# INK-USC/RE-Net

Hardware: AMD Instinct MI355X
Metric: RGCN+GRU encoder triples/s at bs=1024 n_hidden=200 (full training step, both directions) (higher is better)
Workload: dtype f32; 1 GPU; ICEWS18-shaped synthetic stream (seed 999), n_hidden=200, seq_len=10, batch=1024 per GPU, dropout=0.50, fwd+bwd both directions + clip + Adam; parallelism=dp1, global_batch=1024, nodes=99312, edges=288792

## Files before the change

### include/renet_hip.h

```cpp
#ifndef RENET_HIP_H
#define RENET_HIP_H

#include <stddef.h>
#include <stdint.h>

#ifdef __cplusplus
extern "C" {
#endif

#define RENET_OK 0
#define RENET_ERR_BADARG (-1)
#define RENET_ERR_UNSUPPORTED (-2)
#define RENET_ERR_WORKSPACE (-3)

#define RENET_ABI_VERSION 1
int renet_version(void);

int renet_gather_rows(const float* table, const int32_t* idx, int n, int D, float* out, void* stream);
int renet_segment_add(const float* src, const int32_t* order, const int32_t* seg_ptr,
                      const int32_t* seg_target, int U, int D, float* dst, void* stream);
int renet_segment_add2(const float* src0, const float* src1, const int32_t* order, const int32_t* seg_ptr,
                       const int32_t* seg_target, int U, int D, float* dst0, float* dst1, void* stream);

int renet_rgcn_gather(const float* x, int D, const int32_t* row_ptr, const int32_t* col,
// ... 114 lines not shown
                           const int32_t* subj_row, const int32_t* row_ent, const int32_t* row_rel,
                           const int32_t* glob_row, int S, int D, float drop_p, uint64_t seed_x,
                           uint64_t seed_xr, float* X, float* Xr, void* stream);
int renet_bound_parts(size_t total4);
int renet_seq_assemble_fwd_bounds(const float* h2, const float* ent, const float* rel, const float* glob,
                                  const int32_t* subj_row, const int32_t* row_ent, const int32_t* row_rel,
                                  const int32_t* glob_row, int S, int D, float drop_p, uint64_t seed_x,
                                  uint64_t seed_xr, float* X, float* Xr, float* partX, float* partXr, void* stream);
int renet_seq_assemble_bwd(const float* dX, const float* dXr, const int32_t* step_off, int L, int S,
                           int B, int D, float drop_p, uint64_t seed_x, uint64_t seed_xr, float* dRows,
                           float* dEntSeq, float* dRelSeq, void* stream);

size_t renet_gru_workspace(int B, int H);
int renet_gru_fwd(const float* Gi, const int32_t* step_off, int L, int H, const float* Whh,
                  const float* bhh, float* h_last, int out_rows, float* saved, float* workspace,
                  size_t workspace_bytes, void* stream);
int renet_gru_bwd(const float* dh_last, const int32_t* step_off, int L, int H, const float* Whh,
                  const float* saved, float* dGi, float* dGh, float* workspace,
                  size_t workspace_bytes, void* stream);
int renet_gru_fwd_multi(int n, const float* const* Gi, const int32_t* step_off, int L, int H,
                        const float* const* Whh, const float* const* bhh, float* const* h_last, int out_rows,
                        float* const* saved, float* workspace, size_t workspace_bytes, void* stream);
int renet_gru_bwd_multi(int n, const float* const* dh_last, const int32_t* step_off, int L, int H,
                        const float* const* Whh, const float* const* saved, float* const* dGi,
                        float* const* dGh, float* workspace, size_t workspace_bytes, void* stream);
int renet_gru_fwd_layouts(int n, const float* const* Gi, const int32_t* const* step_off, const int* L, int H,
                          const float* const* Whh, const float* const* bhh, float* const* h_last,
                          const int* out_rows, float* const* saved, float* workspace, size_t workspace_bytes,
                          void* stream);
int renet_gru_bwd_layouts(int n, const float* const* dh_last, const int32_t* const* step_off, const int* L, int H,
                          const float* const* Whh, const float* const* saved, float* const* dGi,
                          float* const* dGh, float* workspace, size_t workspace_bytes, void* stream);
int renet_gru_bound_parts(int max_rows);
int renet_gru_bwd_layouts_bounds(int n, const float* const* dh_last, const int32_t* const* step_off, const int* L, int H,
                                 const float* const* Whh, const float* const* saved, float* const* dGi,
                                 float* const* dGh, float* const* bounds, float* workspace, size_t workspace_bytes,
                                 void* stream);
int renet_gru_fwd_layouts_f32(int n, const float* const* Gi, const int32_t* const* step_off, const int* L, int H,
                              const float* const* Whh, const float* const* bhh, float* const* h_last,
                              const int* out_rows, float* const* saved, float* workspace, size_t workspace_bytes,
                              void* stream);
int renet_gru_bwd_layouts_f32(int n, const float* const* dh_last, const int32_t* const* step_off, const int* L, int H,
                              const float* const* Whh, const float* const* saved, float* const* dGi,
                              float* const* dGh, float* workspace, size_t workspace_bytes, void* stream);
int renet_gru_fwd_layouts_bf16(int n, const float* const* Gi, const int32_t* const* step_off, const int* L, int H,
                               const float* const* Whh, const float* const* bhh, float* const* h_last,
                               const int* out_rows, float* const* saved, float* workspace, size_t workspace_bytes,
                               void* stream);
int renet_gru_bwd_layouts_bf16(int n, const float* const* dh_last, const int32_t* const* step_off, const int* L, int H,
                               const float* const* Whh, const float* const* saved, float* const* dGi,
                               float* const* dGh, float* workspace, size_t workspace_bytes, void* stream);

int renet_concat3_fwd(const float* a, const int32_t* ia, const float* hmid, const float* c,
                      const int32_t* ic, int B, int D, float drop_p, uint64_t seed, float* feat,
                      void* stream);
int renet_concat3_fwd_bounds(const float* a, const int32_t* ia, const float* hmid, const float* c,
                             const int32_t* ic, int B, int D, float drop_p, uint64_t seed, float* feat,
                             float* bound_part, void* stream);
int renet_concat3_bwd(const float* dfeat, int B, int D, int parts, float drop_p, uint64_t seed,
                      float* da_rows, float* dhmid, float* dc_rows, void* stream);
int renet_dropout(const float* x, size_t n, float drop_p, uint64_t seed, float* y, void* stream);
int renet_softmax_ce(const float* logits, const int32_t* target, int B, int C, int ld,
                     float grad_scale, float* row_loss, float* dlogits, void* stream);

int renet_segment_pool_fwd(const float* h, const int32_t* seg_ptr, int G, int D, int is_max,
                           float* out, int32_t* argmax, void* stream);
int renet_segment_pool_bwd(const float* dout, const int32_t* seg_ptr, const int32_t* argmax, int G,
                           int D, int is_max, int N, float* dh, void* stream);

size_t renet_adam_workspace(size_t n);
int renet_adam_step(float* p, float* g, float* m, float* v, size_t n, float lr, float beta1, float beta2,
                    float eps, float weight_decay, float max_norm, int step, int zero_grad, float* workspace,
                    size_t workspace_bytes, float* grad_norm_out, void* stream);
int renet_adam_step_scaled(float* p, float* g, float* m, float* v, size_t n, float lr, float beta1, float beta2,
                           float eps, float weight_decay, float max_norm, float grad_scale, int step,
                           int zero_grad, float* workspace, size_t workspace_bytes, float* grad_norm_out,
                           void* stream);

int renet_sumsq_partials(const float* g, size_t n, float* partial, int n_slots, void* stream);
int renet_adam_step_presummed(float* p, float* g, float* m, float* v, size_t n, float lr, float beta1, float beta2,
                              float eps, float weight_decay, float max_norm, float grad_scale, int step, int zero_grad,
                              const float* partial, int n_partial, float* grad_norm_out, void* stream);

int renet_joint_softmax(float* logits, int ld, int n, int R, int N, const float* logits_r, int ld_r,
                        const float* prob_e, void* stream);
size_t renet_topk_workspace(int n);
int renet_topk_positive(const float* x, size_t ldx, int n, int M, int k, float* out_val, int64_t* out_idx,
                        void* workspace, size_t workspace_bytes, void* stream);

int renet_rank_rows(const float* scores, int ld, int n, int C, const int32_t* label, const int32_t* filt_ptr,
                    const int32_t* filt_col, int filtered, int32_t* greater, int32_t* equal, float* row_loss,
                    void* stream);

typedef struct {
    const int32_t *q_s, *q_r, *q_o;
    const int32_t* h_first[2];
    const int32_t* h_count[2];
    const int32_t* snap_t[2];
    const int32_t* snap_ptr[2];
    const int32_t* nbr_o[2];
    const int32_t* times;
    const int32_t* trip_ptr;
    const int32_t *trip_s, *trip_r, *trip_o;
    const int32_t* glob_times;
    int T, n_glob, n_facts, num_ent, num_rels;
} RenetStoreDev;

typedef struct {
    int32_t *node_ent, *node_slot, *row_ptr, *col, *etype;
    float* norm;
    int32_t *heavy_rows, *e_src, *e_dst, *chunk_ptr, *chunk_type, *type_chunk_ptr;
    int32_t *e_src2, *e_dst2, *chunk_ptr2, *chunk_type2, *type_chunk_ptr2;
    int32_t *it_src, *it_type, *grp_ptr;
    int32_t *subj_row, *row_seq, *row_ent, *row_rel, *glob_row;
    int32_t *s_sorted, *r_sorted, *rel_label, *ent_label, *perm, *step_off;
    int32_t* plan_order[4];
    int32_t* plan_seg[4];
    int32_t* plan_target[4];
    int32_t* counts;
    int cap_nodes, cap_edges;
    int32_t* seg_ptr;
} RenetBatchOut;

enum {
    RENET_BB_NNZ = 0, RENET_BB_S, RENET_BB_L, RENET_BB_TB, RENET_BB_FACTS, RENET_BB_N, RENET_BB_NA, RENET_BB_E2,
    RENET_BB_E, RENET_BB_NHEAVY, RENET_BB_NHEAVY_OUT, RENET_BB_NCHUNKS, RENET_BB_NCHUNKS2, RENET_BB_NITEMS,
    RENET_BB_NGROUPS, RENET_BB_NGROUPS_OUT, RENET_BB_NSEG0, RENET_BB_NSEG1, RENET_BB_NSEG2, RENET_BB_NSEG3,
    RENET_BB_ERR, RENET_BB_EOUT,
    RENET_BB_STEP_OFF = 24,
    RENET_BB_NCOUNTS = 64
};
enum { RENET_BB_ERR_TIME = 1, RENET_BB_ERR_GLOB = 2, RENET_BB_ERR_NODES = 4, RENET_BB_ERR_EDGES = 8 };

size_t renet_build_batch_workspace(const RenetStoreDev* store, int B, int cap_nodes, int cap_edges);
int renet_build_batch_both(const RenetStoreDev* store, const int32_t* idx_dev, int B, int seq_len, int heavy_thresh,
                           int group_budget, int chunk, const RenetBatchOut* out, void* workspace,
                           size_t workspace_bytes, void* stream);

typedef struct {
    const int32_t* node_ptr;
    const int32_t* node_ent_all;
    const int32_t* trip_ptr;
    const int32_t *trip_ls, *trip_r, *trip_lo;
    int T, n_nodes, n_facts, num_ent, num_rels;
} RenetFullStoreDev;

size_t renet_build_full_graphs_workspace(const RenetFullStoreDev* store, int G, int cap_nodes, int cap_edges);
int renet_build_full_graphs(const RenetFullStoreDev* store, const int32_t* tidx_dev, int G, int heavy_thresh,
                            int group_items, int chunk, RenetBatchOut* out, void* workspace, size_t workspace_bytes,
                            void* stream);

typedef struct { const int32_t *order, *seg_ptr, *target; int num_segments; } RenetSegPlan;
typedef struct {
    int D, num_ent, T, C2;
    float drop_p;
    const float *ent, *rel;
    const float *w1, *loop1, *w2, *loop2;
    const float *wih, *whh, *bih, *bhh;
    const float *wih_r, *whh_r, *bih_r, *bhh_r;
    const float *lin_w, *lin_b;
    const float *linr_w, *linr_b;
    float *g_ent, *g_rel, *g_w1, *g_loop1, *g_w2, *g_loop2, *g_wih, *g_whh, *g_bih, *g_bhh, *g_wih_r, *g_whh_r, *g_bih_r,
          *g_bhh_r, *g_lin_w, *g_lin_b, *g_linr_w, *g_linr_b;
    const float* glob;
    const void* lin_w_planes;
    size_t lin_w_plane;
// ... 64 lines not shown
```

### re-net_amd/csrc/optim.hip

```cpp
#include "common.h"

namespace {

constexpr int kBlocks = 2048;

__global__ __launch_bounds__(256) void sumsq_partial_kernel(const float4* __restrict__ g, size_t n4,
                                                            const float* __restrict__ g_tail, int tail,
                                                            float* __restrict__ partial) {
    __shared__ float red[4];
    float s = 0.f;
    for (size_t i = (size_t)blockIdx.x * 256 + threadIdx.x; i < n4; i += (size_t)gridDim.x * 256) {
        const float4 v = g[i];
        s += (v.x * v.x + v.y * v.y) + (v.z * v.z + v.w * v.w);
    }
    if (blockIdx.x == 0 && (int)threadIdx.x < tail) s += g_tail[threadIdx.x] * g_tail[threadIdx.x];
#pragma unroll
    for (int o = 32; o > 0; o >>= 1) s += __shfl_xor(s, o);
    if ((threadIdx.x & 63) == 0) red[threadIdx.x >> 6] = s;
    __syncthreads();
    if (threadIdx.x == 0) partial[blockIdx.x] = (red[0] + red[1]) + (red[2] + red[3]);
}

struct AdamCfg {
    float lr, beta1, beta2, eps, wd, max_norm, bc1, bc2_sqrt;
    float grad_scale;
    int zero_grad;
};

__device__ __forceinline__ float adam_one(float& p, float g, float& m, float& v, const AdamCfg& c, float coef) {
    g = g * coef + c.wd * p;
    m = c.beta1 * m + (1.f - c.beta1) * g;
    v = c.beta2 * v + (1.f - c.beta2) * g * g;
    const float denom = sqrtf(v) / c.bc2_sqrt + c.eps;
    p -= (c.lr / c.bc1) * (m / denom);
    return 0.f;
}

__global__ __launch_bounds__(256) void adam_kernel(float* __restrict__ p, float* __restrict__ g,
                                                   float* __restrict__ m, float* __restrict__ v, size_t n,
                                                   const float* __restrict__ partial, int n_partial, AdamCfg c,
                                                   float* __restrict__ norm_out) {
    __shared__ float red[4];
    __shared__ float s_coef;
    float s = 0.f;
    for (int i = threadIdx.x; i < n_partial; i += 256) s += partial[i];
#pragma unroll
    for (int o = 32; o > 0; o >>= 1) s += __shfl_xor(s, o);
    if ((threadIdx.x & 63) == 0) red[threadIdx.x >> 6] = s;
    __syncthreads();
    if (threadIdx.x == 0) {
        const float norm = c.grad_scale * sqrtf((red[0] + red[1]) + (red[2] + red[3]));
        float coef = 1.f;
        if (c.max_norm > 0.f) coef = fminf(c.max_norm / (norm + 1e-6f), 1.f);
        s_coef = coef * c.grad_scale;
        if (blockIdx.x == 0 && norm_out) *norm_out = norm;
    }
    __syncthreads();
    const float coef = s_coef;
    const size_t n4 = n / 4;
    float4* p4 = reinterpret_cast<float4*>(p);
    float4* g4 = reinterpret_cast<float4*>(g);
    float4* m4 = reinterpret_cast<float4*>(m);
    float4* v4 = reinterpret_cast<float4*>(v);
    for (size_t i = (size_t)blockIdx.x * 256 + threadIdx.x; i < n4; i += (size_t)gridDim.x * 256) {
        float4 pp = p4[i], gg = g4[i], mm = m4[i], vv = v4[i];
        adam_one(pp.x, gg.x, mm.x, vv.x, c, coef);
        adam_one(pp.y, gg.y, mm.y, vv.y, c, coef);
        adam_one(pp.z, gg.z, mm.z, vv.z, c, coef);
        adam_one(pp.w, gg.w, mm.w, vv.w, c, coef);
        p4[i] = pp; m4[i] = mm; v4[i] = vv;
        if (c.zero_grad) g4[i] = make_float4(0.f, 0.f, 0.f, 0.f);
    }
    if (blockIdx.x == 0 && threadIdx.x < (n & 3)) {
        const size_t i = n4 * 4 + threadIdx.x;
        float pp = p[i], mm = m[i], vv = v[i];
        adam_one(pp, g[i], mm, vv, c, coef);
        p[i] = pp; m[i] = mm; v[i] = vv;
        if (c.zero_grad) g[i] = 0.f;
    }
}

}

extern "C" {

size_t renet_adam_workspace(size_t n) {
    (void)n;
    return kBlocks * sizeof(float);
}

int renet_adam_step(float* p, float* g, float* m, float* v, size_t n, float lr, float beta1, float beta2,
                    float eps, float weight_decay, float max_norm, int step, int zero_grad, float* workspace,
                    size_t workspace_bytes, float* grad_norm_out, void* stream) {
    return renet_adam_step_scaled(p, g, m, v, n, lr, beta1, beta2, eps, weight_decay, max_norm, 1.f, step, zero_grad,
                                  workspace, workspace_bytes, grad_norm_out, stream);
}

int renet_sumsq_partials(const float* g, size_t n, float* partial, int n_slots, void* stream) {
    if (!g || !partial || n_slots < 1 || n_slots > kBlocks) return RENET_ERR_BADARG;
    if (reinterpret_cast<uintptr_t>(g) & 15) return RENET_ERR_BADARG;
    const size_t n4 = n / 4;
    RENET_LAUNCH(sumsq_partial_kernel, dim3(n_slots), dim3(256), 0, (hipStream_t)stream, (const float4*)g, n4, g + n4 * 4,
                       (int)(n & 3), partial);
    RENET_LAUNCH_CHECK();
    return RENET_OK;
}

static int adam_launch(float* p, float* g, float* m, float* v, size_t n, float lr, float beta1, float beta2, float eps,
                       float weight_decay, float max_norm, float grad_scale, int step, int zero_grad, const float* partial,
                       int n_partial, float* grad_norm_out, hipStream_t st) {
    const size_t n4 = n / 4;
    const int blocks = (int)max((size_t)1, min((size_t)kBlocks, (n4 + 255) / 256));
    AdamCfg c;
    c.lr = lr; c.beta1 = beta1; c.beta2 = beta2; c.eps = eps; c.wd = weight_decay; c.max_norm = max_norm;
    c.bc1 = 1.f - powf(beta1, (float)step);
    c.bc2_sqrt = sqrtf(1.f - powf(beta2, (float)step));
    c.zero_grad = zero_grad;
    c.grad_scale = grad_scale;
    RENET_LAUNCH(adam_kernel, dim3(blocks), dim3(256), 0, st, p, g, m, v, n, partial, n_partial, c, grad_norm_out);
    RENET_LAUNCH_CHECK();
    return RENET_OK;
}

int renet_adam_step_presummed(float* p, float* g, float* m, float* v, size_t n, float lr, float beta1, float beta2,
                              float eps, float weight_decay, float max_norm, float grad_scale, int step, int zero_grad,
                              const float* partial, int n_partial, float* grad_norm_out, void* stream) {
    if (step < 1 || lr < 0.f || beta1 < 0.f || beta1 >= 1.f || beta2 < 0.f || beta2 >= 1.f) return RENET_ERR_BADARG;
    if (n == 0) return RENET_OK;
    if (!partial || n_partial < 1 || n_partial > kBlocks) return RENET_ERR_BADARG;
    if ((reinterpret_cast<uintptr_t>(p) | reinterpret_cast<uintptr_t>(g) | reinterpret_cast<uintptr_t>(m) |
         reinterpret_cast<uintptr_t>(v)) & 15) return RENET_ERR_BADARG;
    return adam_launch(p, g, m, v, n, lr, beta1, beta2, eps, weight_decay, max_norm, grad_scale, step, zero_grad, partial,
                       n_partial, grad_norm_out, (hipStream_t)stream);
}

int renet_adam_step_scaled(float* p, float* g, float* m, float* v, size_t n, float lr, float beta1, float beta2,
                           float eps, float weight_decay, float max_norm, float grad_scale, int step, int zero_grad,
                           float* workspace, size_t workspace_bytes, float* grad_norm_out, void* stream) {
    if (step < 1 || lr < 0.f || beta1 < 0.f || beta1 >= 1.f || beta2 < 0.f || beta2 >= 1.f) return RENET_ERR_BADARG;
    if (n == 0) return RENET_OK;
    if (workspace_bytes < renet_adam_workspace(n)) return RENET_ERR_WORKSPACE;
    if ((reinterpret_cast<uintptr_t>(p) | reinterpret_cast<uintptr_t>(g) | reinterpret_cast<uintptr_t>(m) |
         reinterpret_cast<uintptr_t>(v)) & 15) return RENET_ERR_BADARG;
    hipStream_t st = (hipStream_t)stream;
    const size_t n4 = n / 4;
    const int blocks = (int)max((size_t)1, min((size_t)kBlocks, (n4 + 255) / 256));
    RENET_LAUNCH(sumsq_partial_kernel, dim3(blocks), dim3(256), 0, st, (const float4*)g, n4, g + n4 * 4,
                       (int)(n & 3), workspace);
    RENET_LAUNCH_CHECK();
    return adam_launch(p, g, m, v, n, lr, beta1, beta2, eps, weight_decay, max_norm, grad_scale, step, zero_grad, workspace,
                       blocks, grad_norm_out, st);
}


}
```

### re-net_amd/parallel.py

```python
import os

import torch
import torch.distributed as dist


def flat_layout(params):
    offs, off = [], 0
    for p in params:
        offs.append(off)
        off += (p.numel() + 3) & ~3
    return offs, off


def ordered_params(module, first=()):
    ps = [p for p in module.parameters() if p.requires_grad]
    own = {id(p) for p in ps}
    front, seen = [], set()
    for p in first:
        if id(p) in own and id(p) not in seen:
            front.append(p)
            seen.add(id(p))
    return front + [p for p in ps if id(p) not in seen]


# ... 211 lines not shown
        self.partials_ready = self._done_regions == set(r for r in self.regions() if r[1]) and \
            (self.sumsq_fn is not None or self.stream is None)
        if self.average:
            if fold_scale:
                self.pending_scale = 1.0 / world
            else:
                self.fg.flat.div_(world)
                self.bucket_sumsq = {k: v / float(world) ** 2 for k, v in self.bucket_sumsq.items()}
        for bk in self.buckets:
            bk.count, bk.work = 0, None

    def total_norm(self):
        return float(sum(self.bucket_sumsq.values())) ** 0.5


def shard_indices(perm, step, rank, world, batch_size):
    k = step * world + rank
    n = len(perm)
    start = (k * batch_size) % max(n - batch_size + 1, 1)
    return perm[start:start + batch_size]


class ScalingMode(object):

    MODES = ('weak', 'strong', 'exact')

    def __init__(self, scaling, batch, world, passes='merged'):
        if scaling not in self.MODES:
            raise ValueError('scaling must be one of %s' % (self.MODES,))
        self.scaling, self.world = scaling, int(world)
        self.exact = scaling == 'exact'
        self.rank_batch = int(batch) if scaling in ('weak', 'exact') else max(1, int(batch) // self.world)
        self.global_batch = int(batch) if self.exact else self.rank_batch * self.world
        self.average = not self.exact
        self.passes = 'merged' if self.exact else passes
        self.reported_scaling = 'strong' if scaling in ('strong', 'exact') else 'weak'

    def indices(self, perm, step, rank):
        if self.exact:
            return shard_indices(perm, step, 0, 1, self.rank_batch)
        return shard_indices(perm, step, rank, self.world, self.rank_batch)

    def shard(self, rank):
        return (rank, self.world) if (self.exact and self.world > 1) else None


class FlatParams(object):

    def __init__(self, module, first=()):
        self.params = ordered_params(module, first)
        self.offsets, total = flat_layout(self.params)
        dev = self.params[0].device
        self.flat = torch.zeros(total, device=dev, dtype=torch.float32)
        self.numel = total
        with torch.no_grad():
            for p, off in zip(self.params, self.offsets):
                n = p.numel()
                self.flat[off:off + n].copy_(p.data.reshape(-1))
                p.data = self.flat[off:off + n].view_as(p)


class HipAdam(object):

    def __init__(self, module, lr=1e-3, betas=(0.9, 0.999), eps=1e-8, weight_decay=0.0, max_norm=0.0):
        import renet_hip as K
        self.K = K
        self._module = module
        names = dict((id(p), n) for n, p in module.named_parameters())
        head = [p for n, p in module.named_parameters() if n in ('linear.weight', 'linear.bias')]
        mid = [p for n, p in module.named_parameters() if n.startswith(('encoder.', 'encoder_r.'))] if head else []
        if os.environ.get('RENET_REDUCER_BUCKETS', '3') == '2':
            mid = []
        self.params = FlatParams(module, first=head + mid)
        self.grads = FlatGrads(module, first=head + mid)
        self.m = torch.zeros_like(self.params.flat)
        self.v = torch.zeros_like(self.params.flat)
        self.lr, self.betas, self.eps, self.wd, self.max_norm = lr, betas, eps, weight_decay, max_norm
        self.t = 0
        self.norm = torch.zeros(1, device=self.m.device, dtype=torch.float32)
        self.reducer = None
        self._hook = None
        self._weights = [p for p in self.params.params if p.dim() == 2]
        K.register_weights(self._weights)
        if head:
            mid_names = tuple(names[id(p)] for p in mid)
            self._part = torch.zeros(self.PART_SLOTS * 4, device=self.m.device, dtype=torch.float32)
            self.reducer = OverlapReducer(self.grads, self.grads.span(('linear.weight', 'linear.bias'), module), head,
                                          mid_span=self.grads.span(mid_names, module) if mid else None, mid_params=mid,
                                          sumsq_fn=self._region_sumsq if self.m.is_cuda else None)
            import ops
            self._hook = ops.register_grad_done_hook(head + mid, self.reducer.on_grad_done,
                                                     wanted=lambda r=self.reducer: r.armed and r.active())

    PART_SLOTS = 512

    def _region_sumsq(self, k, region):
        self.K.sumsq_partials(region, self._part, k * self.PART_SLOTS, self.PART_SLOTS)

    def close(self):
        if self._hook is not None:
            import ops
            ops.unregister_grad_done_hook(self._hook)
            self._hook = None
        if getattr(self, '_weights', None):
            self.K.unregister_weights(self._weights)
            self._weights = []

    def __del__(self):
        try:
            self.close()
        except Exception:
            pass

    def step_scope(self, head_passes=2, average=True):
        return _StepScope(self, head_passes, average)

    @staticmethod
    def sync_grads():
        import ops
        ops.join_deferred()

    def step(self):
        scale = 1.0
        import ops
        ops.join_deferred()
        if self.reducer is not None:
            self.reducer.finish(fold_scale=True)
            scale = self.reducer.pending_scale
        elif dist.is_available() and dist.is_initialized() and dist.get_world_size() > 1:
            dist.all_reduce(self.grads.flat, op=dist.ReduceOp.SUM)
            scale = 1.0 / dist.get_world_size()
        self.t += 1
        pre = None
        if self.reducer is not None and self.reducer.partials_ready and self.reducer.sumsq_fn is not None:
            pre = (self._part, self.PART_SLOTS * len(self.reducer.regions()))
        self.K.adam_step(self.params.flat, self.grads.flat, self.m, self.v, self.lr, self.betas[0], self.betas[1],
                         self.eps, self.wd, self.max_norm, self.t, True, self.norm, grad_scale=scale, presummed=pre)
        self.K.weights_changed()
        with self.K.gemm_mode(getattr(self._module, 'gemm_mode', None)):
            self.K.prefetch_weight_bounds(self.params.flat.device)


class _StepScope(object):
    def __init__(self, opt, head_passes, average):
        self.opt, self.head_passes, self.average = opt, head_passes, average

    def __enter__(self):
        if self.opt.reducer is not None:
            self.opt.reducer.begin_step(self.head_passes, self.average)
        import ops
        self._defer_old = ops.DEFER_WEIGHT_GRADS
        ops.DEFER_WEIGHT_GRADS = os.environ.get('RENET_DEFER_GRADS', '1') != '0'
        return self.opt

    def __exit__(self, exc_type, exc, tb):
        import ops
        ops.DEFER_WEIGHT_GRADS = self._defer_old
        ops.join_deferred()
        r = self.opt.reducer
        if r is not None and r.armed:
            r.armed = False
            for bk in r.buckets:
                if bk.work is not None:
                    r._wait(bk)
                bk.count = 0
        return False
```

### re-net_amd/renet_hip.py

```python
import contextlib
import ctypes
import functools
import os
import threading
import weakref

import torch

_HERE = os.path.dirname(os.path.abspath(__file__))
LIB_PATH = os.environ.get('RENET_HIP_LIB', os.path.join(_HERE, 'csrc', 'librenet_hip.so'))

_lib = None

c_int = ctypes.c_int
c_float = ctypes.c_float
c_void_p = ctypes.c_void_p
c_size_t = ctypes.c_size_t
c_u64 = ctypes.c_uint64

_GEMM_ARGS = [c_int, c_int, c_int, c_int, c_int, c_float, c_void_p, c_int, c_void_p, c_int,
              c_float, c_void_p, c_int, c_void_p, c_int, c_void_p, c_size_t, c_void_p]
_RGCN_BWD_W_ARGS = [c_void_p, c_void_p, c_void_p, c_void_p, c_void_p, c_void_p, c_int,
                    c_void_p, c_int, c_int, c_int, c_void_p, c_float, c_void_p, c_size_t, c_void_p]
_GRU_FWD_LAYOUTS_ARGS = [c_int, c_void_p, c_void_p, c_void_p, c_int, c_void_p, c_void_p, c_void_p,
# ... 51 lines not shown
    'renet_bf16_zero_padding': (c_int, [c_void_p, c_int, c_int, c_int, c_int, c_void_p]),
    'renet_seq_assemble_fwd_bf16': (c_int, [c_void_p, c_void_p, c_void_p, c_void_p, c_void_p, c_void_p, c_void_p,
                                            c_void_p, c_int, c_int, c_float, c_u64, c_u64, c_void_p, c_int, c_void_p,
                                            c_int, c_int, c_void_p]),
    'renet_softmax_ce_bf16': (c_int, [c_void_p, c_void_p, c_int, c_int, c_int, c_float, c_void_p, c_void_p, c_int, c_int,
                                      c_void_p]),
    'renet_gru_bwd_layouts_bf16out': (c_int, [c_int, c_void_p, c_void_p, c_void_p, c_int, c_void_p, c_void_p, c_void_p,
                                              c_void_p, c_int, c_void_p, c_size_t, c_void_p]),
    'renet_colsum_bf16': (c_int, [c_void_p, c_int, c_int, c_int, c_void_p, c_float, c_void_p, c_size_t, c_void_p]),
    'renet_scale_bf16_by_device_scalar': (c_int, [c_void_p, c_size_t, c_void_p, c_void_p]),
    'renet_planes_elems': (c_size_t, [c_int, c_int]),
    'renet_pack_planes': (c_int, [c_void_p, c_int, c_int, c_int, c_int, c_void_p, c_void_p]),
    'renet_gemm_planes': (c_int, [c_int, c_int, c_int, c_int, c_int, c_float, c_void_p, c_void_p, c_int, c_size_t,
                                  c_void_p, c_int, c_size_t, c_float, c_void_p, c_int, c_void_p, c_void_p, c_int,
                                  c_void_p, c_size_t, c_void_p]),
    'renet_softmax_ce_planes': (c_int, [c_void_p, c_void_p, c_int, c_int, c_int, c_float, c_void_p, c_void_p, c_size_t,
                                        c_int, c_int, c_void_p]),
    'renet_step_workspace': (c_size_t, [c_void_p, c_void_p]),
    'renet_step_forward': (c_int, [c_void_p, c_void_p, c_void_p, c_void_p, c_void_p]),
    'renet_step_backward': (c_int, [c_void_p, c_void_p, c_void_p, c_void_p, c_int, c_void_p, c_void_p, c_void_p]),
    'renet_add_inplace': (c_int, [c_void_p, c_void_p, c_size_t, c_void_p]),
    'renet_zero': (c_int, [c_void_p, c_size_t, c_void_p]),
    'renet_colsum_workspace': (c_size_t, [c_int, c_int]),
    'renet_colsum': (c_int, [c_void_p, c_int, c_int, c_int, c_void_p, c_float, c_void_p, c_size_t, c_void_p]),
    'renet_scale_by_device_scalar': (c_int, [c_void_p, c_size_t, c_void_p, c_void_p]),
    'renet_scale_by_device_scalar_bound': (c_int, [c_void_p, c_size_t, c_void_p, c_float, c_void_p, c_void_p]),
    'renet_seq_assemble_fwd': (c_int, [c_void_p, c_void_p, c_void_p, c_void_p, c_void_p, c_void_p, c_void_p,
                                       c_void_p, c_int, c_int, c_float, c_u64, c_u64, c_void_p, c_void_p,
                                       c_void_p]),
    'renet_seq_assemble_fwd_bounds': (c_int, [c_void_p, c_void_p, c_void_p, c_void_p, c_void_p, c_void_p, c_void_p,
                                              c_void_p, c_int, c_int, c_float, c_u64, c_u64, c_void_p, c_void_p,
                                              c_void_p, c_void_p, c_void_p]),
    'renet_seq_assemble_bwd': (c_int, [c_void_p, c_void_p, c_void_p, c_int, c_int, c_int, c_int, c_float,
                                       c_u64, c_u64, c_void_p, c_void_p, c_void_p, c_void_p]),
    'renet_gru_workspace': (c_size_t, [c_int, c_int]),
    'renet_gru_fwd': (c_int, [c_void_p, c_void_p, c_int, c_int, c_void_p, c_void_p, c_void_p, c_int, c_void_p,
                              c_void_p, c_size_t, c_void_p]),
    'renet_gru_bwd': (c_int, [c_void_p, c_void_p, c_int, c_int, c_void_p, c_void_p, c_void_p, c_void_p,
                              c_void_p, c_size_t, c_void_p]),
    'renet_gru_fwd_multi': (c_int, [c_int, c_void_p, c_void_p, c_int, c_int, c_void_p, c_void_p, c_void_p,
                                    c_int, c_void_p, c_void_p, c_size_t, c_void_p]),
    'renet_gru_bwd_multi': (c_int, [c_int, c_void_p, c_void_p, c_int, c_int, c_void_p, c_void_p, c_void_p,
                                    c_void_p, c_void_p, c_size_t, c_void_p]),
    'renet_gru_fwd_layouts': (c_int, _GRU_FWD_LAYOUTS_ARGS),
    'renet_gru_bwd_layouts': (c_int, _GRU_BWD_LAYOUTS_ARGS),
    'renet_gru_bound_parts': (c_int, [c_int]),
    'renet_gru_bwd_layouts_bounds': (c_int, [c_int, c_void_p, c_void_p, c_void_p, c_int, c_void_p, c_void_p, c_void_p,
                                             c_void_p, c_void_p, c_void_p, c_size_t, c_void_p]),
    'renet_gru_fwd_layouts_f32': (c_int, _GRU_FWD_LAYOUTS_ARGS),
    'renet_gru_bwd_layouts_f32': (c_int, _GRU_BWD_LAYOUTS_ARGS),
    'renet_gru_fwd_layouts_bf16': (c_int, _GRU_FWD_LAYOUTS_ARGS),
    'renet_gru_bwd_layouts_bf16': (c_int, _GRU_BWD_LAYOUTS_ARGS),
    'renet_concat3_fwd': (c_int, [c_void_p, c_void_p, c_void_p, c_void_p, c_void_p, c_int, c_int, c_float,
                                  c_u64, c_void_p, c_void_p]),
    'renet_concat3_fwd_bounds': (c_int, [c_void_p, c_void_p, c_void_p, c_void_p, c_void_p, c_int, c_int, c_float,
                                         c_u64, c_void_p, c_void_p, c_void_p]),
    'renet_concat3_bwd': (c_int, [c_void_p, c_int, c_int, c_int, c_float, c_u64, c_void_p, c_void_p,
                                  c_void_p, c_void_p]),
    'renet_dropout': (c_int, [c_void_p, c_size_t, c_float, c_u64, c_void_p, c_void_p]),
    'renet_softmax_ce': (c_int, [c_void_p, c_void_p, c_int, c_int, c_int, c_float, c_void_p, c_void_p,
                                 c_void_p]),
    'renet_joint_softmax': (c_int, [c_void_p, c_int, c_int, c_int, c_int, c_void_p, c_int, c_void_p, c_void_p]),
    'renet_rank_rows': (c_int, [c_void_p, c_int, c_int, c_int, c_void_p, c_void_p, c_void_p, c_int, c_void_p, c_void_p,
                                c_void_p, c_void_p]),
    'renet_topk_workspace': (c_size_t, [c_int]),
    'renet_topk_positive': (c_int, [c_void_p, c_size_t, c_int, c_int, c_int, c_void_p, c_void_p, c_void_p, c_size_t,
                                    c_void_p]),
    'renet_build_batch_workspace': (c_size_t, [c_void_p, c_int, c_int, c_int]),
    'renet_build_batch_both': (c_int, [c_void_p, c_void_p, c_int, c_int, c_int, c_int, c_int, c_void_p, c_void_p, c_size_t,
                                       c_void_p]),
    'renet_build_full_graphs_workspace': (c_size_t, [c_void_p, c_int, c_int, c_int]),
    'renet_build_full_graphs': (c_int, [c_void_p, c_void_p, c_int, c_int, c_int, c_int, c_void_p, c_void_p, c_size_t,
                                        c_void_p]),
    'renet_adam_workspace': (c_size_t, [c_size_t]),
    'renet_adam_step': (c_int, [c_void_p, c_void_p, c_void_p, c_void_p, c_size_t, c_float, c_float, c_float, c_float,
                                c_float, c_float, c_int, c_int, c_void_p, c_size_t, c_void_p, c_void_p]),
    'renet_adam_step_scaled': (c_int, [c_void_p, c_void_p, c_void_p, c_void_p, c_size_t, c_float, c_float, c_float,
                                       c_float, c_float, c_float, c_float, c_int, c_int, c_void_p, c_size_t, c_void_p,
                                       c_void_p]),
    'renet_sumsq_partials': (c_int, [c_void_p, c_size_t, c_void_p, c_int, c_void_p]),
    'renet_adam_step_presummed': (c_int, [c_void_p, c_void_p, c_void_p, c_void_p, c_size_t, c_float, c_float, c_float,
                                          c_float, c_float, c_float, c_float, c_int, c_int, c_void_p, c_int, c_void_p,
                                          c_void_p]),
    'renet_host_filter_edges': (ctypes.c_int64, [c_void_p] * 5 + [ctypes.c_int64, ctypes.c_int64, c_void_p, c_void_p,
                                                 ctypes.c_int64, c_void_p, c_void_p, c_void_p, c_void_p]),
    'renet_host_filter_edges_sparse': (ctypes.c_int64, [c_void_p] * 7 + [ctypes.c_int64, ctypes.c_int64, c_void_p,
                                                        c_void_p, ctypes.c_int64, c_void_p, c_void_p, c_void_p,
                                                        c_void_p]),
    'renet_host_node_sets': (ctypes.c_int64, [ctypes.c_int64] + [c_void_p] * 5 + [ctypes.c_int64, ctypes.c_int64]
                             + [c_void_p] * 7),
    'renet_host_type_chunks': (ctypes.c_int64, [ctypes.c_int64, c_void_p, c_void_p, c_void_p, ctypes.c_int64,
                                                ctypes.c_int64, ctypes.c_int64] + [c_void_p] * 6),
    'renet_host_edge_layouts': (None, [ctypes.c_int64, ctypes.c_int64, c_void_p, c_void_p, c_void_p, ctypes.c_int64,
                                       ctypes.c_int64, ctypes.c_int64] + [c_void_p] * 12),
    'renet_host_segplan': (ctypes.c_int64, [c_void_p, ctypes.c_int64, ctypes.c_int64, c_void_p, c_void_p, c_void_p]),
    'renet_host_gather_items': (ctypes.c_int64, [ctypes.c_int64, c_void_p, c_void_p, c_void_p, ctypes.c_int64,
                                                 ctypes.c_int64, ctypes.c_int64] + [c_void_p] * 5),
    'renet_segment_pool_fwd': (c_int, [c_void_p, c_void_p, c_int, c_int, c_int, c_void_p, c_void_p, c_void_p]),
    'renet_segment_pool_bwd': (c_int, [c_void_p, c_void_p, c_void_p, c_int, c_int, c_int, c_int, c_void_p,
                                       c_void_p]),
}

EXPORTS = sorted(_SIGNATURES)


class RenetHipError(RuntimeError):
    pass


class _Bound(object):
    """The bound entry points (attribute per symbol)."""


def _exact_arity(fn, name, n):
    def call(*a):
        if len(a) != n:
            raise RenetHipError('%s takes %d arguments, %d given' % (name, n, len(a)))
        return fn(*a)
    call.__name__ = name
    return call


def lib():
    global _lib
    if _lib is None:
        if not os.path.isfile(LIB_PATH):
            raise RenetHipError('librenet_hip.so not built (%s); run `python re-net_amd/build.py` '
                                '-- there is no fallback path' % LIB_PATH)
        L = ctypes.CDLL(LIB_PATH)
        ns = _Bound()
        for name, (res, args) in _SIGNATURES.items():
            fn = getattr(L, name)
            fn.restype = res
            fn.argtypes = args
            setattr(ns, name, _exact_arity(fn, name, len(args)))
        if ns.renet_version() != 1:
            raise RenetHipError('ABI version mismatch')
        ns._cdll = L
        _lib = ns
    return _lib


def _check(rc, what):
    if rc != 0:
        raise RenetHipError('%s failed with code %d' % (what, rc))


def _dev_ptr(dtype, default_name, t, name=None):
    if t is None:
        return None
    if not (t.is_cuda and t.dtype == dtype and t.is_contiguous()):
        raise RenetHipError('%s must be a contiguous %s device tensor' % (name or default_name, str(dtype)[6:]))
    return t.data_ptr()


_f32 = functools.partial(_dev_ptr, torch.float32, 'tensor')
_i32 = functools.partial(_dev_ptr, torch.int32, 'index')


_raw_stream = getattr(torch._C, '_cuda_getCurrentRawStream', None)


def _stream():
    if _raw_stream is not None:
        return _raw_stream(torch.cuda.current_device())
    return torch.cuda.current_stream().cuda_stream
# ... 958 lines not shown
    dc = torch.empty(b, d, device=dfeat.device, dtype=torch.float32) if parts == 3 else None
    _check(lib().renet_concat3_bwd(_f32(dfeat), b, d, parts, float(drop_p), int(seed), _f32(da), _f32(dh),
                                   _f32(dc), _stream()), 'concat3_bwd')
    return da, dh, dc


def dropout(x, drop_p, seed):
    y = torch.empty_like(x)
    _check(lib().renet_dropout(_f32(x), x.numel(), float(drop_p), int(seed), _f32(y), _stream()), 'dropout')
    return y


def softmax_ce(logits, target, grad_scale, want_grad, row_loss=None):
    b, c = logits.shape
    if row_loss is None:
        row_loss = torch.empty(b, device=logits.device, dtype=torch.float32)
    _check(lib().renet_softmax_ce(logits.data_ptr(), _i32(target), b, c, _ld(logits), float(grad_scale),
                                  _f32(row_loss), logits.data_ptr() if want_grad else None, _stream()),
           'softmax_ce')
    return row_loss


def rank_rows(scores, label, filt_ptr=None, filt_col=None, filtered=True, want_loss=True):
    if not (scores.is_cuda and scores.dtype == torch.float32 and scores.dim() == 2):
        raise RenetHipError('rank_rows needs a 2-D float32 device tensor')
    n, c = scores.shape
    if label.numel() != n or (filt_ptr is not None and (filt_col is None or filt_ptr.numel() != n + 1)):
        raise RenetHipError('rank_rows: shape mismatch')
    counts = torch.empty(2, n, device=scores.device, dtype=torch.int32)
    row_loss = torch.empty(n, device=scores.device, dtype=torch.float32) if want_loss else None
    t0 = _timed()
    _check(lib().renet_rank_rows(scores.data_ptr(), max(_ld(scores), c) if n == 1 else _ld(scores), n, c, _i32(label),
                                 _i32(filt_ptr), _i32(filt_col), int(bool(filtered)), counts[0].data_ptr(),
                                 counts[1].data_ptr(), _f32(row_loss), _stream()), 'rank_rows')
    _timed_end(t0, 'rank_rows', nbytes=float(n * c * 4))
    return counts, row_loss


def joint_softmax(logits, num_rels, logits_r, prob_e):
    nr, n_ent = logits.shape
    n = nr // num_rels
    if nr != n * num_rels or tuple(logits_r.shape) != (n, num_rels) or prob_e.numel() != n:
        raise RenetHipError('joint_softmax: shape mismatch')
    _check(lib().renet_joint_softmax(logits.data_ptr(), _ld(logits), n, num_rels, n_ent, logits_r.data_ptr(),
                                     _ld(logits_r), _f32(prob_e), _stream()), 'joint_softmax')
    return logits


def topk_positive(x, k):
    if not (x.is_cuda and x.dtype == torch.float32 and x.dim() == 2 and x.stride(1) == 1):
        raise RenetHipError('topk_positive needs a 2-D float32 device tensor with unit inner stride')
    n, m = x.shape
    vals = torch.empty(n, k, device=x.device, dtype=torch.float32)
    idx = torch.empty(n, k, device=x.device, dtype=torch.int64)
    nbytes = lib().renet_topk_workspace(n)
    ws = torch.empty(nbytes // 4 + 1, device=x.device, dtype=torch.int32)
    _check(lib().renet_topk_positive(x.data_ptr(), x.stride(0) if n > 1 else m, n, m, int(k), vals.data_ptr(),
                                     idx.data_ptr(), ws.data_ptr(), nbytes, _stream()), 'topk_positive')
    return vals, idx


def segment_pool_fwd(h, seg_ptr, num_graphs, is_max):
    d = h.shape[1]
    out = torch.empty(num_graphs, d, device=h.device, dtype=torch.float32)
    arg = torch.empty(num_graphs, d, device=h.device, dtype=torch.int32)
    _check(lib().renet_segment_pool_fwd(_f32(h), _i32(seg_ptr), num_graphs, d, int(is_max), _f32(out),
                                        _i32(arg), _stream()), 'segment_pool_fwd')
    return out, arg


def segment_pool_bwd(dout, seg_ptr, arg, num_graphs, is_max, n):
    d = dout.shape[1]
    dh = torch.empty(n, d, device=dout.device, dtype=torch.float32)
    _check(lib().renet_segment_pool_bwd(_f32(dout), _i32(seg_ptr), _i32(arg), num_graphs, d, int(is_max), n,
                                        _f32(dh), _stream()), 'segment_pool_bwd')
    return dh


def sumsq_partials(g, partial, slot0, n_slots):
    _check(lib().renet_sumsq_partials(_f32(g), g.numel(), partial.data_ptr() + 4 * slot0, int(n_slots), _stream()),
           'sumsq_partials')


def adam_step(p, g, m, v, lr, beta1, beta2, eps, weight_decay, max_norm, step, zero_grad=True, norm_out=None,
              grad_scale=1.0, presummed=None):
    n = p.numel()
    if presummed is not None:
        part, n_part = presummed
        _check(lib().renet_adam_step_presummed(_f32(p), _f32(g), _f32(m), _f32(v), n, float(lr), float(beta1), float(beta2),
                                               float(eps), float(weight_decay), float(max_norm), float(grad_scale),
                                               int(step), int(zero_grad), _f32(part), int(n_part), _f32(norm_out),
                                               _stream()), 'adam_step_presummed')
        return
    nbytes = lib().renet_adam_workspace(n)
    ws = torch.empty(nbytes // 4, device=p.device, dtype=torch.float32)
    _check(lib().renet_adam_step_scaled(_f32(p), _f32(g), _f32(m), _f32(v), n, float(lr), float(beta1), float(beta2),
                                        float(eps), float(weight_decay), float(max_norm), float(grad_scale), int(step),
                                        int(zero_grad), ws.data_ptr(), nbytes, _f32(norm_out), _stream()), 'adam_step')
```

### re-net_amd/step_plan.py

```python
import ctypes
import os
import weakref

import torch
from torch.autograd import Function

import ops
import renet_hip as K

ENABLED = os.environ.get('RENET_STEP_PLAN', '1') != '0'

_cache = weakref.WeakKeyDictionary()


def _slot(net):
    c = _cache.get(net)
    if c is None:
        c = _cache[net] = {}
    return c

_P = ctypes.c_void_p
_I = ctypes.c_int


# ... 127 lines not shown
            p = getattr(g, n)
        c = SegPlanC(K._i32(p.order), K._i32(p.seg_ptr), K._i32(p.target), int(p.num_segments))
        setattr(b, n, c)
        plans.append(p)
    prep._step_batch = (b, tens, plans, (it_src_t, it_type_t, col_t, e_src_t))
    return b


_events = {}
_hook_streams = {}


def _side_stream(device):
    if not (ops.SIDE_STREAM and device.type == 'cuda'):
        return None
    key = device.index if device.index is not None else torch.cuda.current_device()
    st = ops._side_streams.get(key)
    if st is None:
        st = ops._side_streams[key] = torch.cuda.Stream(device=device)
    return st


def _head_event(device, which=0):
    key = (device.index if device.index is not None else torch.cuda.current_device(), which)
    ev = _events.get(key)
    if ev is None:
        ev = torch.cuda.Event()
        ev.record()
        _events[key] = ev
        _hook_streams[key] = torch.cuda.Stream(device=device)
    return ev, _hook_streams[key]


class StepFn(Function):

    @staticmethod
    def forward(ctx, net, prep, row_tap, *params):
        dev = net.ent_embeds.device
        g = prep.g
        p = float(net.drop_p) if net.training else 0.0
        with ops.shared_graph_seeds(getattr(prep, 'sharded', False) or ops.SHARED_GRAPH_SEEDS):
            s_r1 = ops.next_seed(graph_site=True) if p > 0 else 0
            s_r2 = ops.next_seed(graph_site=True) if p > 0 else 0
            s_x, s_xr = (ops.next_seed(), ops.next_seed()) if p > 0 else (0, 0)
        s_h1, s_h2 = (ops.next_seed(), ops.next_seed()) if p > 0 else (0, 0)
        planes = K.weight_planes(params[14]) if K.use_planes(params[14], params[14].shape[0]) else None
        m = _model_struct(net, params, planes)
        m.glob = K._f32(g.glob, 'global embeddings')
        b = _batch_struct(prep)
        lib = K.lib()
        nbytes = lib.renet_step_workspace(ctypes.addressof(m), ctypes.addressof(b))
        if nbytes == 0:
            raise K.RenetHipError('renet_step_workspace rejected the model / batch')
        ws = torch.empty(nbytes, device=dev, dtype=torch.uint8)
        scale = 2.0 * getattr(prep, 'share', 1.0)
        bb = prep.b
        s1, s2 = float(scale) / bb, float(scale) * 0.1 / bb
        rl = torch.empty(2 * bb, device=dev, dtype=torch.float32)
        side = _side_stream(dev)
        r = StepRunC(int(s_r1), int(s_r2), int(s_x), int(s_xr), int(s_h1), int(s_h2), s1, s2, ws.data_ptr(), nbytes,
                     K._stream(), side.cuda_stream if side is not None else None)
        nl = ctypes.c_int(0)
        K._check(lib.renet_step_forward(ctypes.addressof(m), ctypes.addressof(b), ctypes.addressof(r), rl.data_ptr(),
                                        ctypes.addressof(nl)), 'renet_step_forward')
        ctx.net, ctx.prep, ctx.m, ctx.b, ctx.r, ctx.ws, ctx.planes = net, prep, m, b, r, ws, planes
        ctx.consumed = False
        ctx.launches = nl.value
        ctx.gemm_mode = K.current_mode()
        ctx.side = side
        net.aggregator.last_batch = g
        StepFn.last_launches = [nl.value, 0]
        if row_tap is not None:
            row_tap.append((rl.detach(), s1, s2))
        return torch.dot(rl, ops._loss_weight_vector(bb, s1, s2, dev))

    @staticmethod
    def backward(ctx, g):
        if ctx.consumed:
            raise RuntimeError('StepFn: the saved CE gradients were consumed by the first backward pass; a second pass over '
                               'the same graph is not supported')
        ctx.consumed = True
        params = model_params(ctx.net)
        m, b, r = ctx.m, ctx.b, ctx.r
        missing = [i for i, p in enumerate(params) if not _grad_ok(p)]
        fresh = [None] * len(params)
        if missing:
            if any(params[i].grad is not None for i in missing):
                raise RuntimeError('StepFn: a parameter has an unusable .grad (non-contiguous / wrong dtype); set '
                                   'RENET_STEP_PLAN=0')
            offs, tot = [], 0
            for i in missing:
                offs.append(tot)
                tot += (params[i].numel() + 3) & ~3
            flat = torch.zeros(tot, device=params[0].device, dtype=torch.float32)
            for i, o in zip(missing, offs):
                fresh[i] = flat[o:o + params[i].numel()].view_as(params[i])
        for i, (n, p) in enumerate(zip(_PARAMS, params)):
            setattr(m, 'g_' + n, (fresh[i] if fresh[i] is not None else p.grad).data_ptr())
        dev = ctx.net.ent_embeds.device
        side = ctx.side
        r.stream = K._stream()
        r.side_stream = side.cuda_stream if side is not None else None
        defer = bool(ops.DEFER_WEIGHT_GRADS and side is not None and not missing)
        lin_w, lin_b = params[14], params[15]
        hooked = (ops.hooks_wanted(lin_w) or ops.hooks_wanted(lin_b)) and not missing
        ev = hs = ev2 = hs2 = None
        if hooked:
            ev, hs = _head_event(dev)
        gru_params = params[6:14]
        hooked_gru = not missing and any(ops.hooks_wanted(p) for p in gru_params)
        if hooked_gru:
            ev2, hs2 = _head_event(dev, 1)
        g = g.contiguous()
        nl = ctypes.c_int(0)
        lib = K.lib()
        K._check(lib.renet_step_backward(ctypes.addressof(m), ctypes.addressof(b), ctypes.addressof(r), K._f32(g),
                                         int(defer), ev.cuda_event if ev is not None else None,
                                         ev2.cuda_event if ev2 is not None else None, ctypes.addressof(nl)),
                 'renet_step_backward')
        StepFn.last_launches[1] = nl.value
        if hooked_gru:
            hs2.wait_event(ev2)
            with torch.cuda.stream(hs2):
                for p in gru_params:
                    ops.grad_done(p)
        if hooked:
            hs.wait_event(ev)
            with torch.cuda.stream(hs):
                ops.grad_done(lin_w)
                ops.grad_done(lin_b)
        keep = (ctx.ws, ctx.prep, ctx.planes, m, b, g)
        if defer:
            ops._deferred.append((torch.cuda.current_stream(dev), side, keep))
        ctx.ws = None
        return (None, None, None) + tuple(fresh)


StepFn.last_launches = [0, 0]
```

Before: 385,100 triples/s.

## Fuse bf16 three-plane split of head weight into Adam step

Adds an Adam kernel variant in which a subset of blocks updates the output-head weight tile by tile and writes its updated values directly as three bf16 residual planes in the tiled layout the GEMM uses. The remaining blocks update the rest of the flat parameter buffer and skip the emitted regions. The optimizer then registers these planes as the weight's cached split, so the separate re-split pass over the head weight after each step can be skipped. The cost is a more complex Adam kernel with per-element ownership checks and a heuristic block partition. The step-plan backward also re-fetches the plane pointers so it picks up the fresh planes.

```diff
diff --git a/include/renet_hip.h b/include/renet_hip.h
--- a/include/renet_hip.h
+++ b/include/renet_hip.h
@@ -220,6 +220,20 @@
                               float eps, float weight_decay, float max_norm, float grad_scale, int step, int zero_grad,
                               const float* partial, int n_partial, float* grad_norm_out, void* stream);
 
+#define RENET_EMIT_T16_PLANES 1
+typedef struct RenetAdamEmit {
+    size_t offset;
+    int rows, cols;
+    int format;
+    int ld;
+    size_t plane;
+    void* dst;
+} RenetAdamEmit;
+int renet_adam_step_emit(float* p, float* g, float* m, float* v, size_t n, float lr, float beta1, float beta2, float eps,
+                         float weight_decay, float max_norm, float grad_scale, int step, int zero_grad,
+                         const float* partial, int n_partial, float* workspace, size_t workspace_bytes,
+                         float* grad_norm_out, const RenetAdamEmit* emit, int n_emit, void* stream);
+
 int renet_joint_softmax(float* logits, int ld, int n, int R, int N, const float* logits_r, int ld_r,
                         const float* prob_e, void* stream);
 size_t renet_topk_workspace(int n);
diff --git a/re-net_amd/csrc/optim.hip b/re-net_amd/csrc/optim.hip
--- a/re-net_amd/csrc/optim.hip
+++ b/re-net_amd/csrc/optim.hip
@@ -36,10 +36,48 @@
     return 0.f;
 }
 
+constexpr int kMaxEmit = 4;
+
+struct EmitRegion {
+    size_t off, end;
+    int rows, cols;
+    int nbc;
+    int item_end;
+    int tcc;
+    __bf16* dst;
+    size_t plane;
+};
+
+struct EmitList {
+    int n, items;
+    EmitRegion r[kMaxEmit];
+};
+
+typedef float f32x2 __attribute__((ext_vector_type(2)));
+typedef __bf16 bf16x2 __attribute__((ext_vector_type(2)));
+
+__device__ __forceinline__ void emit_t16(const float4& x, __bf16* dst, size_t plane) {
+    f32x2 lo = {x.x, x.y}, hi = {x.z, x.w};
+#pragma unroll
+    for (int t = 0; t < 3; ++t) {
+        const bf16x2 blo = __builtin_convertvector(lo, bf16x2);
+        const bf16x2 bhi = __builtin_convertvector(hi, bf16x2);
+        uint2 w;
+        w.x = __builtin_bit_cast(uint32_t, blo);
+        w.y = __builtin_bit_cast(uint32_t, bhi);
+        *reinterpret_cast<uint2*>(dst + (size_t)t * plane) = w;
+        if (t < 2) {
+            lo -= __builtin_convertvector(blo, f32x2);
+            hi -= __builtin_convertvector(bhi, f32x2);
+        }
+    }
+}
+
+template <bool EMIT>
 __global__ __launch_bounds__(256) void adam_kernel(float* __restrict__ p, float* __restrict__ g,
                                                    float* __restrict__ m, float* __restrict__ v, size_t n,
                                                    const float* __restrict__ partial, int n_partial, AdamCfg c,
-                                                   float* __restrict__ norm_out) {
+                                                   float* __restrict__ norm_out, EmitList em, int emit_blocks) {
     __shared__ float red[4];
     __shared__ float s_coef;
     float s = 0.f;
@@ -62,7 +100,40 @@
     float4* g4 = reinterpret_cast<float4*>(g);
     float4* m4 = reinterpret_cast<float4*>(m);
     float4* v4 = reinterpret_cast<float4*>(v);
-    for (size_t i = (size_t)blockIdx.x * 256 + threadIdx.x; i < n4; i += (size_t)gridDim.x * 256) {
+    if (EMIT && (int)blockIdx.x < emit_blocks) {
+        const int lane = threadIdx.x & 63;
+        for (int it = blockIdx.x; it < em.items; it += emit_blocks) {
+            int d = 0, first = 0;
+#pragma unroll
+            for (int k = 0; k + 1 < kMaxEmit; ++k)
+                if (k + 1 < em.n && it >= em.r[k].item_end) { d = k + 1; first = em.r[k].item_end; }
+            const EmitRegion& R = em.r[d];
+            const int local = it - first;
+            const int tr = local / R.nbc;
+            const int tc = (local - tr * R.nbc) * 4 + (threadIdx.x >> 6);
+            const int row = tr * 16 + (lane >> 2), col = tc * 16 + (lane & 3) * 4;
+            if (row >= R.rows || col >= R.cols) continue;
+            const size_t i = (R.off + (size_t)row * R.cols + col) >> 2;
+            float4 pp = p4[i], gg = g4[i], mm = m4[i], vv = v4[i];
+            adam_one(pp.x, gg.x, mm.x, vv.x, c, coef);
+            adam_one(pp.y, gg.y, mm.y, vv.y, c, coef);
+            adam_one(pp.z, gg.z, mm.z, vv.z, c, coef);
+            adam_one(pp.w, gg.w, mm.w, vv.w, c, coef);
+            p4[i] = pp; m4[i] = mm; v4[i] = vv;
+            if (c.zero_grad) g4[i] = make_float4(0.f, 0.f, 0.f, 0.f);
+            emit_t16(pp, R.dst + renet_t16_off(row, col, R.tcc), R.plane);
+        }
+        return;
+    }
+    const int fb = EMIT ? (int)blockIdx.x - emit_blocks : (int)blockIdx.x;
+    const int nfb = EMIT ? (int)gridDim.x - emit_blocks : (int)gridDim.x;
+    for (size_t i = (size_t)fb * 256 + threadIdx.x; i < n4; i += (size_t)nfb * 256) {
+        if (EMIT) {
+            bool owned = false;
+#pragma unroll
+            for (int k = 0; k < kMaxEmit; ++k) owned |= k < em.n && i * 4 >= em.r[k].off && i * 4 < em.r[k].end;
+            if (owned) continue;
+        }
         float4 pp = p4[i], gg = g4[i], mm = m4[i], vv = v4[i];
         adam_one(pp.x, gg.x, mm.x, vv.x, c, coef);
         adam_one(pp.y, gg.y, mm.y, vv.y, c, coef);
@@ -71,7 +142,7 @@
         p4[i] = pp; m4[i] = mm; v4[i] = vv;
         if (c.zero_grad) g4[i] = make_float4(0.f, 0.f, 0.f, 0.f);
     }
-    if (blockIdx.x == 0 && threadIdx.x < (n & 3)) {
+    if (fb == 0 && threadIdx.x < (n & 3)) {
         const size_t i = n4 * 4 + threadIdx.x;
         float pp = p[i], mm = m[i], vv = v[i];
         adam_one(pp, g[i], mm, vv, c, coef);
@@ -106,9 +177,34 @@
     return RENET_OK;
 }
 
+static int make_emit_list(const RenetAdamEmit* emit, int n_emit, size_t n, EmitList& em) {
+    em.n = 0; em.items = 0;
+    for (int k = 0; k < kMaxEmit; ++k) em.r[k] = EmitRegion{0, 0, 0, 0, 1, 0, 0, nullptr, 0};
+    if (n_emit < 0 || n_emit > kMaxEmit || (n_emit > 0 && !emit)) return RENET_ERR_BADARG;
+    for (int k = 0; k < n_emit; ++k) {
+        const RenetAdamEmit& e = emit[k];
+        if (e.format != RENET_EMIT_T16_PLANES) return RENET_ERR_UNSUPPORTED;
+        if (e.rows < 1 || e.cols < 1 || (e.cols & 3) || (e.offset & 3) || !e.dst) return RENET_ERR_BADARG;
+        const size_t count = (size_t)e.rows * e.cols;
+        if (count > 0x7fffffffu || e.offset > n || count > n - e.offset) return RENET_ERR_BADARG;
+        const size_t rp = ((size_t)e.rows + 15) & ~(size_t)15, cp = ((size_t)e.cols + 15) & ~(size_t)15;
+        if (e.ld < 16 || (e.ld & 15) || (size_t)e.ld < cp || e.plane < rp * (size_t)e.ld) return RENET_ERR_BADARG;
+        if (reinterpret_cast<uintptr_t>(e.dst) & 7) return RENET_ERR_BADARG;
+        for (int j = 0; j < k; ++j)
+            if (e.offset < em.r[j].end && em.r[j].off < e.offset + count) return RENET_ERR_BADARG;
+        const size_t nbc = ((size_t)e.cols + 63) / 64, items = nbc * (rp / 16);
+        if (items > (size_t)0x7fffffff - em.items) return RENET_ERR_UNSUPPORTED;
+        em.items += (int)items;
+        em.r[k] = EmitRegion{e.offset, e.offset + count, e.rows, e.cols, (int)nbc, em.items, e.ld >> 4,
+                             reinterpret_cast<__bf16*>(e.dst), e.plane};
+        em.n = k + 1;
+    }
+    return RENET_OK;
+}
+
 static int adam_launch(float* p, float* g, float* m, float* v, size_t n, float lr, float beta1, float beta2, float eps,
                        float weight_decay, float max_norm, float grad_scale, int step, int zero_grad, const float* partial,
-                       int n_partial, float* grad_norm_out, hipStream_t st) {
+                       int n_partial, float* grad_norm_out, hipStream_t st, const EmitList* em = nullptr) {
     const size_t n4 = n / 4;
     const int blocks = (int)max((size_t)1, min((size_t)kBlocks, (n4 + 255) / 256));
     AdamCfg c;
@@ -117,7 +213,19 @@
     c.bc2_sqrt = sqrtf(1.f - powf(beta2, (float)step));
     c.zero_grad = zero_grad;
     c.grad_scale = grad_scale;
-    RENET_LAUNCH(adam_kernel, dim3(blocks), dim3(256), 0, st, p, g, m, v, n, partial, n_partial, c, grad_norm_out);
+    if (em && em->n > 0) {
+        size_t owned = 0;
+        for (int k = 0; k < em->n; ++k) owned += em->r[k].end - em->r[k].off;
+        const double we = 1.25 * (double)owned, wf = (double)(n - owned);
+        int eb = (int)(we / (we + wf) * blocks + 0.5);
+        eb = max(1, min(min(eb, em->items), blocks));
+        const int fb = max(1, blocks - eb);
+        RENET_LAUNCH(adam_kernel<true>, dim3(eb + fb), dim3(256), 0, st, p, g, m, v, n, partial, n_partial, c, grad_norm_out,
+                     *em, eb);
+    } else {
+        RENET_LAUNCH(adam_kernel<false>, dim3(blocks), dim3(256), 0, st, p, g, m, v, n, partial, n_partial, c,
+                     grad_norm_out, EmitList{}, 0);
+    }
     RENET_LAUNCH_CHECK();
     return RENET_OK;
 }
@@ -152,5 +260,31 @@
                        blocks, grad_norm_out, st);
 }
 
-
-}
+int renet_adam_step_emit(float* p, float* g, float* m, float* v, size_t n, float lr, float beta1, float beta2, float eps,
+                         float weight_decay, float max_norm, float grad_scale, int step, int zero_grad,
+                         const float* partial, int n_partial, float* workspace, size_t workspace_bytes,
+                         float* grad_norm_out, const RenetAdamEmit* emit, int n_emit, void* stream) {
+    if (step < 1 || lr < 0.f || beta1 < 0.f || beta1 >= 1.f || beta2 < 0.f || beta2 >= 1.f) return RENET_ERR_BADARG;
+    if (n == 0) return n_emit == 0 ? RENET_OK : RENET_ERR_BADARG;
+    if ((reinterpret_cast<uintptr_t>(p) | reinterpret_cast<uintptr_t>(g) | reinterpret_cast<uintptr_t>(m) |
+         reinterpret_cast<uintptr_t>(v)) & 15) return RENET_ERR_BADARG;
+    EmitList em;
+    const int e = make_emit_list(emit, n_emit, n, em);
+    if (e != RENET_OK) return e;
+    hipStream_t st = (hipStream_t)stream;
+    if (partial) {
+        if (n_partial < 1 || n_partial > kBlocks) return RENET_ERR_BADARG;
+    } else {
+        if (!workspace || workspace_bytes < renet_adam_workspace(n)) return RENET_ERR_WORKSPACE;
+        const size_t n4 = n / 4;
+        n_partial = (int)max((size_t)1, min((size_t)kBlocks, (n4 + 255) / 256));
+        RENET_LAUNCH(sumsq_partial_kernel, dim3(n_partial), dim3(256), 0, st, (const float4*)g, n4, g + n4 * 4,
+                     (int)(n & 3), workspace);
+        RENET_LAUNCH_CHECK();
+        partial = workspace;
+    }
+    return adam_launch(p, g, m, v, n, lr, beta1, beta2, eps, weight_decay, max_norm, grad_scale, step, zero_grad, partial,
+                       n_partial, grad_norm_out, st, &em);
+}
+
+}
diff --git a/re-net_amd/parallel.py b/re-net_amd/parallel.py
--- a/re-net_amd/parallel.py
+++ b/re-net_amd/parallel.py
@@ -317,6 +317,8 @@
         self._hook = None
         self._weights = [p for p in self.params.params if p.dim() == 2]
         K.register_weights(self._weights)
+        self._head_w = next((p for n, p in module.named_parameters() if n == 'linear.weight'), None)
+        self._head_planes = None
         if head:
             mid_names = tuple(names[id(p)] for p in mid)
             self._part = torch.zeros(self.PART_SLOTS * 4, device=self.m.device, dtype=torch.float32)
@@ -354,6 +356,18 @@
     def sync_grads():
         import ops
         ops.join_deferred()
+
+    def _head_emit(self):
+        K, w = self.K, self._head_w
+        if w is None or not K.use_planes(w, w.shape[0]) or w.shape[1] % 4:
+            return None, None
+        off = next((o for p, o in zip(self.params.params, self.params.offsets) if p is w), None)
+        if off is None or off % 4 or w.data_ptr() != self.params.flat.data_ptr() + 4 * off:
+            return None, None
+        mat = self._head_planes
+        if mat is None or mat.shape != tuple(w.shape) or mat.p.device != w.device:
+            mat = self._head_planes = K.planes_empty(w.shape[0], w.shape[1], w.device, zero=True)
+        return [K.adam_emit_planes(off, mat)], mat
 
     def step(self):
         scale = 1.0
@@ -369,9 +383,14 @@
         pre = None
         if self.reducer is not None and self.reducer.partials_ready and self.reducer.sumsq_fn is not None:
             pre = (self._part, self.PART_SLOTS * len(self.reducer.regions()))
+        with self.K.gemm_mode(getattr(self._module, 'gemm_mode', None)):
+            emit, mat = self._head_emit()
         self.K.adam_step(self.params.flat, self.grads.flat, self.m, self.v, self.lr, self.betas[0], self.betas[1],
-                         self.eps, self.wd, self.max_norm, self.t, True, self.norm, grad_scale=scale, presummed=pre)
+                         self.eps, self.wd, self.max_norm, self.t, True, self.norm, grad_scale=scale, presummed=pre,
+                         emit=emit)
         self.K.weights_changed()
+        if mat is not None:
+            self.K.note_weight_planes(self._head_w, mat)
         with self.K.gemm_mode(getattr(self._module, 'gemm_mode', None)):
             self.K.prefetch_weight_bounds(self.params.flat.device)
 
diff --git a/re-net_amd/renet_hip.py b/re-net_amd/renet_hip.py
--- a/re-net_amd/renet_hip.py
+++ b/re-net_amd/renet_hip.py
@@ -157,6 +157,9 @@
     'renet_adam_step_presummed': (c_int, [c_void_p, c_void_p, c_void_p, c_void_p, c_size_t, c_float, c_float, c_float,
                                           c_float, c_float, c_float, c_float, c_int, c_int, c_void_p, c_int, c_void_p,
                                           c_void_p]),
+    'renet_adam_step_emit': (c_int, [c_void_p, c_void_p, c_void_p, c_void_p, c_size_t, c_float, c_float, c_float, c_float,
+                                     c_float, c_float, c_float, c_int, c_int, c_void_p, c_int, c_void_p, c_size_t, c_void_p,
+                                     c_void_p, c_int, c_void_p]),
     'renet_host_filter_edges': (ctypes.c_int64, [c_void_p] * 5 + [ctypes.c_int64, ctypes.c_int64, c_void_p, c_void_p,
                                                  ctypes.c_int64, c_void_p, c_void_p, c_void_p, c_void_p]),
     'renet_host_filter_edges_sparse': (ctypes.c_int64, [c_void_p] * 7 + [ctypes.c_int64, ctypes.c_int64, c_void_p,
@@ -1281,9 +1284,33 @@
            'sumsq_partials')
 
 
+EMIT_T16_PLANES = 1
+
+
+class AdamEmitC(ctypes.Structure):
+    _fields_ = [('offset', c_size_t), ('rows', c_int), ('cols', c_int), ('format', c_int), ('ld', c_int),
+                ('plane', c_size_t), ('dst', c_void_p)]
+
+
+def adam_emit_planes(offset, mat):
+    return AdamEmitC(int(offset), mat.R, mat.C, EMIT_T16_PLANES, mat.p.shape[2], mat.plane, mat.p.data_ptr())
+
+
 def adam_step(p, g, m, v, lr, beta1, beta2, eps, weight_decay, max_norm, step, zero_grad=True, norm_out=None,
-              grad_scale=1.0, presummed=None):
+              grad_scale=1.0, presummed=None, emit=None):
     n = p.numel()
+    if emit:
+        part, n_part = presummed if presummed is not None else (None, 0)
+        ws, nbytes = None, 0
+        if presummed is None:
+            nbytes = lib().renet_adam_workspace(n)
+            ws = torch.empty(nbytes // 4, device=p.device, dtype=torch.float32)
+        arr = (AdamEmitC * len(emit))(*emit)
+        _check(lib().renet_adam_step_emit(_f32(p), _f32(g), _f32(m), _f32(v), n, float(lr), float(beta1), float(beta2),
+                                          float(eps), float(weight_decay), float(max_norm), float(grad_scale), int(step),
+                                          int(zero_grad), _f32(part), int(n_part), _f32(ws), nbytes, _f32(norm_out),
+                                          ctypes.addressof(arr), len(emit), _stream()), 'adam_step_emit')
+        return
     if presummed is not None:
         part, n_part = presummed
         _check(lib().renet_adam_step_presummed(_f32(p), _f32(g), _f32(m), _f32(v), n, float(lr), float(beta1), float(beta2),
diff --git a/re-net_amd/step_plan.py b/re-net_amd/step_plan.py
--- a/re-net_amd/step_plan.py
+++ b/re-net_amd/step_plan.py
@@ -233,6 +233,9 @@
         ctx.consumed = True
         params = model_params(ctx.net)
         m, b, r = ctx.m, ctx.b, ctx.r
+        if ctx.planes is not None:
+            ctx.planes = K.weight_planes(params[14])
+            m.lin_w_planes, m.lin_w_plane, m.lin_w_ld = ctx.planes.p.data_ptr(), ctx.planes.plane, ctx.planes.p.shape[2]
         missing = [i for i, p in enumerate(params) if not _grad_ok(p)]
         fresh = [None] * len(params)
         if missing:
```

Measured after the change: 384,200 triples/s. No clear change (-0.2%).
